# srvk/eesen

Measured on AMD Instinct MI355X. Metric: CTC training frames/sec (whole node), 4x512 BiLSTM, higher is better.
Workload: dtype f32

## Files before the change

### eesen_amd/csrc/kernels.h

```cpp
#pragma once
#include "common.h"

namespace eesen {

struct GemmBound {
  const float* p = nullptr;
  int per_index = 0;
};
void gemm_f32(hipStream_t st, bool a_kc, bool b_kc, int M, int N, int K, float alpha, const float* A, int lda,
              const float* B, int ldb, float beta, float* C, int ldc, const float* bias, float* ws,
              size_t ws_floats, int extra_lds_bytes = 0,
              bool bf16_operands = false,
              GemmBound bound_a = {}, GemmBound bound_b = {});

constexpr int kDefaultGemmMode = 2;
int gemm_mode();
void set_gemm_mode(int mode);
void amax_abs(hipStream_t st, const float* P, long rows, int cols, int ld, float* out);
void amax_abs_accumulate(hipStream_t st, const float* P, long rows, int cols, int ld, float* out);
constexpr int kAmaxBlocks = 512;
void amax_rows_cols(hipStream_t st, const float* P, long rows, int cols, int ld, float* out_rows, float* out_cols, float* ws);

#ifndef EESEN_SHARDS
#define EESEN_SHARDS 8
// ... 29 lines not shown
  int poll_delay = 0;
  int poll_raw = 0;
  unsigned* milestone = nullptr;
  int milestone_step = 0;
  int xcd_map = 1, fwd_mux = 1, bwd_q4 = 1, bwd_ksplit = 1, bwd_mux = 1;
  int fwd_t16_small = 1;
  int fwd_narrow2 = 1;
  int bwd_q4_st8 = 1;
  int fwd_bf16 = 0;
  int fwd_split = 0;
  int fwd_f16 = 0;
  const float* wm_amax = nullptr;
  int bwd_f16 = 0;
  unsigned char* DGH = nullptr;
  float* EX = nullptr;
};
size_t lstm_bwd_planes_ex_floats(const LstmLayerDev& L);
float handoff_flight_ns();
void set_gpu_share(int n);
int gpu_share_value();
void wait_for_word(hipStream_t st, const unsigned* word, unsigned target, unsigned* err, double limit_s = 2.0);
void lstm_fwd_step(hipStream_t st, const LstmLayerDev& L, int step);
void lstm_bwd_step(hipStream_t st, const LstmLayerDev& L, int step, const float* dY, int lddy, float* DG, float* DCF);
bool lstm_fwd_persistent(hipStream_t st, const LstmLayerDev& L, unsigned* cnt, unsigned* err, int spin_limit,
                         unsigned long long* trace = nullptr, hipEvent_t after_reset = nullptr);
void dropout_mask(hipStream_t st, float* out, long rows, int cols, int ld, float p, unsigned long long seed, bool per_column);
void activation_rows(hipStream_t st, bool tanh_, const float* x, int ldx, float* y, int ldy, long rows, int cols);
void activation_diff_rows(hipStream_t st, bool tanh_, const float* y, int ldy, float* d, int ldd, long rows, int cols);
void mul_elements(hipStream_t st, const float* a, int lda, const float* m, int ldm, float* out, int ldo, long rows, int cols);
void lstm_fwd_persistent_geometry(const LstmLayerDev& L, int* nblk, int* nz, int* units_per_wg = nullptr);
// ... 8 lines not shown
  int seq_tile = 0;
  int units = 0;
  int windows = 0;
  int grid[3] = {0, 0, 0};
  int wgs = 0;
  int wgs_per_cu = 0;
  int vgprs = 0, lds = 0;
  int free_vgprs = -1;
  bool light = false;
  int cpw = 0, stq = 0, chunk = 0, xchg = 0;
  const void* fn = nullptr;
};
RecPlan lstm_fwd_plan(const LstmLayerDev& L);
RecPlan lstm_bwd_plan(const LstmLayerDev& L, bool assume_px);
bool lstm_bwd_persistent(hipStream_t st, const LstmLayerDev& L, const float* dY, int lddy, float* DG, unsigned* cnt,
                         unsigned* err, int spin_limit, unsigned long long* trace = nullptr);
void lstm_bias_peep_grads(hipStream_t st, const LstmLayerDev& L, const float* DG, float* bias_grad, float* peep_grad,
                          float* ws, size_t ws_floats);
size_t lstm_bias_peep_ws_floats(int T, int S, int H, int ndir);

void col_sums(hipStream_t st, const float* M, int rows, int cols, int ld, float* out, float* ws, size_t ws_floats);
size_t col_sums_ws_floats(int rows, int cols);

void softmax_rows(hipStream_t st, const float* x, int ldx, float* y, int ldy, int rows, int K);
void log_rows(hipStream_t st, const float* in, int ldi, float* out, int ldo, int rows, int K);
void ctc_alpha_beta(hipStream_t st, const float* logp, int ld, int T, int S, int Lpad, const int* labx, const int* lens,
                    const int* lablens, float* alpha, float* beta, float* pzx, int waves = 0);
int ctc_sweep_waves(int Lpad, int waves = 0);
void ctc_error_diff(hipStream_t st, const float* probs, int ld, int T, int S, int K, int Lpad, int Lmax, const int* lens,
                    const int* lablens, const int* labx, const float* alpha, const float* beta,
                    const float* pzx, float* diff, int ldd);
void log_sub_prior(hipStream_t st, float* m, int ld, int rows, int K, bool apply_log, const float* log_prior, float prior_scale);
void row_argmax(hipStream_t st, const float* m, int ld, int rows, int K, int* ids);
// ... 22 lines not shown
```

### eesen_amd/csrc/lstm.hip

```cpp
#include "kernels.h"

namespace eesen {
namespace {

typedef float f32x4 __attribute__((ext_vector_type(4)));
constexpr int NW = 8;

#ifndef EESEN_RCP
#define EESEN_RCP(x) __builtin_amdgcn_rcpf(x)
#endif
__device__ __forceinline__ float sigmoidf_(float x) { return EESEN_RCP(1.f + __expf(-x)); }
__device__ __forceinline__ float tanhf_(float x) { return 1.f - 2.f * EESEN_RCP(1.f + __expf(2.f * x)); }

__device__ __forceinline__ void ld8(const float* __restrict__ row, int k, int kmax, bool ok, float (&v)[8]) {
  float4 a = make_float4(0.f, 0.f, 0.f, 0.f), b = a;
  if (ok && k < kmax) a = *reinterpret_cast<const float4*>(row + k);
  if (ok && k + 4 < kmax) b = *reinterpret_cast<const float4*>(row + k + 4);
  v[0] = a.x; v[1] = a.y; v[2] = a.z; v[3] = a.w;
  v[4] = b.x; v[5] = b.y; v[6] = b.z; v[7] = b.w;
}

template <int CPW>
__global__ __launch_bounds__(NW * 64) void lstm_fwd_step_kernel(LstmLayerDev L, int step) {
  __shared__ __attribute__((aligned(16))) float red[NW][32][20];
// ... 168 lines not shown
    dcm = dc * L.rmask[cofs];
    if (L.drop_mode == 2) dcx = dcm;
  }
  float df = f * (1.f - f) * (dcx * c_p);
  float di = i * (1.f - i) * (dcm * g);
  float dg = (1.f - g * g) * (dcm * i);
  float carry = dcx * f;
  if (t >= len) { dg = di = df = dob = 0.f; carry = 0.f; }
  *reinterpret_cast<float4*>(DG + gofs) = make_float4(dg, di, df, dob);
  DCF[(size_t)s_e * ldY + dir * H + u_e] = carry;
  asm volatile("" ::"v"(pf.x), "v"(pf.y), "v"(pf.z), "v"(pf.w), "v"(pf1), "v"(pf2));
}

constexpr int RED_RB = 64;

__global__ __launch_bounds__(256) void lstm_bias_peep_pass1(const float* __restrict__ DG, const float* __restrict__ C,
                                                            int R, int S, int H, int ndir, float* __restrict__ ws) {
  __shared__ float sm[4][64][7];
  const int ul = threadIdx.x & 63, rl = threadIdx.x >> 6;
  const int NU = ndir * H;
  const int gu = blockIdx.x * 64 + ul;
  const int rows_per = (R + RED_RB - 1) / RED_RB;
  const int rbeg = blockIdx.y * rows_per, rend = min(R, rbeg + rows_per);
  float acc[7] = {0.f, 0.f, 0.f, 0.f, 0.f, 0.f, 0.f};
  if (gu < NU) {
    const int dir = gu / H;
    const size_t cs_shift = dir == 0 ? 0 : 2 * (size_t)S;
    for (int r = rbeg + rl; r < rend; r += 4) {
      const float4 d = *reinterpret_cast<const float4*>(DG + (size_t)r * NU * 4 + (size_t)gu * 4);
      const float cs = C[((size_t)r + cs_shift) * NU + gu];
      const float c1 = C[((size_t)r + S) * NU + gu];
      acc[0] += d.x; acc[1] += d.y; acc[2] += d.z; acc[3] += d.w;
      acc[4] += d.y * cs; acc[5] += d.z * cs; acc[6] += d.w * c1;
    }
  }
#pragma unroll
  for (int q = 0; q < 7; ++q) sm[rl][ul][q] = acc[q];
  __syncthreads();
  if (rl == 0 && gu < NU) {
#pragma unroll
    for (int q = 0; q < 7; ++q)
      ws[((size_t)blockIdx.y * NU + gu) * 7 + q] = sm[0][ul][q] + sm[1][ul][q] + sm[2][ul][q] + sm[3][ul][q];
  }
}

__global__ __launch_bounds__(256) void lstm_bias_peep_pass2(const float* __restrict__ ws, int H, int ndir,
                                                            float* __restrict__ bias_grad, float* __restrict__ peep_grad) {
  const int NU = ndir * H;
  const int idx = blockIdx.x * blockDim.x + threadIdx.x;
  if (idx >= NU * 7) return;
  const int gu = idx / 7, q = idx % 7;
  float s = 0.f;
  for (int rb = 0; rb < RED_RB; ++rb) s += ws[((size_t)rb * NU + gu) * 7 + q];
  if (q < 4) {
    bias_grad[(size_t)gu * 4 + q] = s;
  } else {
    const int dir = gu / H, u = gu % H;
    peep_grad[((size_t)dir * 3 + (q - 4)) * H + u] = s;
  }
}

__global__ __launch_bounds__(256) void col_sums_pass1(const float* __restrict__ M, int rows, int cols, int ld,
                                                      float* __restrict__ ws) {
  __shared__ float sm[4][64];
  const int cl = threadIdx.x & 63, rl = threadIdx.x >> 6;
  const int c = blockIdx.x * 64 + cl;
  const int rows_per = (rows + RED_RB - 1) / RED_RB;
  const int rbeg = blockIdx.y * rows_per, rend = min(rows, rbeg + rows_per);
  float acc = 0.f;
  if (c < cols)
    for (int r = rbeg + rl; r < rend; r += 4) acc += M[(size_t)r * ld + c];
  sm[rl][cl] = acc;
  __syncthreads();
// ... 18 lines not shown
void lstm_fwd_step(hipStream_t st, const LstmLayerDev& L, int step) {
  dim3 grid(L.H / 4, L.ndir, cdiv(L.S, 32)), block(NW * 64);
  switch (std::min(4, pick_cpw((L.H + 31) / 32))) {
    case 1: hipLaunchKernelGGL(lstm_fwd_step_kernel<1>, grid, block, 0, st, L, step); break;
    case 2: hipLaunchKernelGGL(lstm_fwd_step_kernel<2>, grid, block, 0, st, L, step); break;
    default: hipLaunchKernelGGL(lstm_fwd_step_kernel<4>, grid, block, 0, st, L, step); break;
  }
}

void lstm_bwd_step(hipStream_t st, const LstmLayerDev& L, int step, const float* dY, int lddy, float* DG, float* DCF) {
  dim3 grid(cdiv(L.H, 16), L.ndir, cdiv(L.S, 16)), block(NW * 64);
  if (pick_cpw((4 * L.H + 31) / 32) <= 1) hipLaunchKernelGGL(lstm_bwd_step_kernel<1>, grid, block, 0, st, L, step, dY, lddy, DG, DCF);
  else hipLaunchKernelGGL(lstm_bwd_step_kernel<2>, grid, block, 0, st, L, step, dY, lddy, DG, DCF);
}

size_t lstm_bias_peep_ws_floats(int T, int S, int H, int ndir) { return (size_t)RED_RB * ndir * H * 7; }

void lstm_bias_peep_grads(hipStream_t st, const LstmLayerDev& L, const float* DG, float* bias_grad, float* peep_grad,
                          float* ws, size_t ws_floats) {
  const int NU = L.ndir * L.H, R = L.T * L.S;
  EESEN_REQUIRE(ws_floats >= lstm_bias_peep_ws_floats(L.T, L.S, L.H, L.ndir), EESEN_ERR_INVALID, "reduction workspace too small");
  hipLaunchKernelGGL(lstm_bias_peep_pass1, dim3(cdiv(NU, 64), RED_RB), dim3(256), 0, st, DG, (const float*)L.C, R, L.S,
                     L.H, L.ndir, ws);
  check_launch("lstm_bias_peep_pass1");
  hipLaunchKernelGGL(lstm_bias_peep_pass2, dim3(cdiv(NU * 7, 256)), dim3(256), 0, st, (const float*)ws, L.H, L.ndir,
                     bias_grad, peep_grad);
  check_launch("lstm_bias_peep_pass2");
}

size_t col_sums_ws_floats(int rows, int cols) { return (size_t)RED_RB * cols; }

void col_sums(hipStream_t st, const float* M, int rows, int cols, int ld, float* out, float* ws, size_t ws_floats) {
  EESEN_REQUIRE(ws_floats >= col_sums_ws_floats(rows, cols), EESEN_ERR_INVALID, "reduction workspace too small");
  hipLaunchKernelGGL(col_sums_pass1, dim3(cdiv(cols, 64), RED_RB), dim3(256), 0, st, M, rows, cols, ld, ws);
  check_launch("col_sums_pass1");
  hipLaunchKernelGGL(col_sums_pass2, dim3(cdiv(cols, 256)), dim3(256), 0, st, (const float*)ws, cols, out);
  check_launch("col_sums_pass2");
}

}
```

### eesen_amd/csrc/lstm_persistent.hip

```cpp
#include "kernels.h"

#include <atomic>
#include <map>
#include <mutex>

namespace eesen {
namespace {

typedef float f32x4 __attribute__((ext_vector_type(4)));
constexpr int NW = 8;
constexpr int kSc1 = 16;

#define EESEN_RCP(x) __builtin_amdgcn_rcpf(x)
__device__ __forceinline__ float sigmoidf_(float x) { return EESEN_RCP(1.f + __expf(-x)); }
__device__ __forceinline__ float tanhf_(float x) { return 1.f - 2.f * EESEN_RCP(1.f + __expf(2.f * x)); }

__device__ __forceinline__ __amdgpu_buffer_rsrc_t make_rsrc(const float* base) {
  return __builtin_amdgcn_make_buffer_rsrc(const_cast<float*>(base), 0, 0x7fffffff, 0x00020000);
}
__device__ __forceinline__ float ld1(__amdgpu_buffer_rsrc_t r, unsigned byte_off) {
  return __builtin_bit_cast(float, __builtin_amdgcn_raw_buffer_load_b32(r, byte_off, 0, 0));
}
constexpr int EESEN_POLL_WAVE = 7;
constexpr int EESEN_POLL_SLEEP = 1;
// ... 896 lines not shown
  float dcf = 0.f, dn_i = 0.f, dn_f = 0.f;
  const size_t gcol = (size_t)dir * K4 + u_e * 4;
  const size_t ycol = (size_t)dir * H + u_e;
  float4 gt = make_float4(0.f, 0.f, 0.f, 0.f);
  float dy = 0.f, c_t = 0.f, c_p = 0.f;
  {
    const int t0 = dir == 0 ? T - 1 : 0, tp0 = dir == 0 ? t0 - 1 : t0 + 1;
    if (e_ok) {
      gt = *reinterpret_cast<const float4*>(L.G + (size_t)(t0 * S + s_e) * ldG + gcol);
      dy = dY[(size_t)(t0 * S + s_e) * lddy + ycol];
      c_t = L.C[(size_t)((t0 + 1) * S + s_e) * ldY + ycol];
      c_p = L.C[(size_t)((tp0 + 1) * S + s_e) * ldY + ycol];
    }
  }
  const __amdgpu_buffer_rsrc_t rDG = make_rsrc(DG);
  __syncthreads();
  for (int step = 0; step < T; ++step) {
    const int t = dir == 0 ? T - 1 - step : step;
    const int tn = dir == 0 ? t + 1 : t - 1;
    f32x4 ac[HS][2];
#pragma unroll
    for (int hs = 0; hs < HS; ++hs) { ac[hs][0] = f32x4{0.f, 0.f, 0.f, 0.f}; ac[hs][1] = f32x4{0.f, 0.f, 0.f, 0.f}; }
    f32x4 a4[HS][P];
    const float4 gtc = gt;
    const float dyc = dy, ctc = c_t, cpc = c_p;
    EESEN_STAMP(0);
    if (step > 0) {
      if (wave == EESEN_POLL_WAVE) {
        const bool go = wait_counters(my_cnt, nblk, (unsigned)step, err, spin_limit, lane, L.poll_delay);
        if (lane == 0) s_go = go ? 1 : 0;
// ... 36 lines not shown
              if (h == 0)      { ac[hs][0] = __builtin_amdgcn_mfma_f32_4x4x1f32(a4[hs][p][r], w0[r], ac[hs][0], 3, 0, 0); ac[hs][1] = __builtin_amdgcn_mfma_f32_4x4x1f32(a4[hs][p][r], w1[r], ac[hs][1], 3, 1, 0); }
              else if (h == 1) { ac[hs][0] = __builtin_amdgcn_mfma_f32_4x4x1f32(a4[hs][p][r], w0[r], ac[hs][0], 3, 2, 0); ac[hs][1] = __builtin_amdgcn_mfma_f32_4x4x1f32(a4[hs][p][r], w1[r], ac[hs][1], 3, 3, 0); }
              else if (h == 2) { ac[hs][0] = __builtin_amdgcn_mfma_f32_4x4x1f32(a4[hs][p][r], w0[r], ac[hs][0], 3, 4, 0); ac[hs][1] = __builtin_amdgcn_mfma_f32_4x4x1f32(a4[hs][p][r], w1[r], ac[hs][1], 3, 5, 0); }
              else             { ac[hs][0] = __builtin_amdgcn_mfma_f32_4x4x1f32(a4[hs][p][r], w0[r], ac[hs][0], 3, 6, 0); ac[hs][1] = __builtin_amdgcn_mfma_f32_4x4x1f32(a4[hs][p][r], w1[r], ac[hs][1], 3, 7, 0); }
            }
          }
        }
      }
    }
#pragma unroll
    for (int hs = 0; hs < HS; ++hs)
#pragma unroll
      for (int i = 0; i < 4; ++i) red[wave][hs * 8 + ks * 4 + i][ab * 4 + x] = ac[hs][0][i] + ac[hs][1][i];
    EESEN_STAMP(2);
    __syncthreads();
    if (e_ok) {
      float ra[NW], rb[NW];
#pragma unroll
      for (int w = 0; w < NW; ++w) { ra[w] = red[w][(es >> 2) * 8 + (es & 3)][eu]; rb[w] = red[w][(es >> 2) * 8 + 4 + (es & 3)][eu]; }
      __builtin_amdgcn_sched_barrier(0);
      float dm = dyc;
#pragma unroll
      for (int w = 0; w < NW; ++w) dm += ra[w] + rb[w];
      const float g = gtc.x, i = gtc.y, f = gtc.z, o = gtc.w;
      const float h = tanhf_(ctc);
      const float dh = (1.f - h * h) * (dm * o);
      float dob = o * (1.f - o) * (dm * h);
      const float dc = dh + dcf + dn_i * p_i + dn_f * p_f + dob * p_o;
      float df = f * (1.f - f) * (dc * cpc);
      float di = i * (1.f - i) * (dc * g);
      float dg = (1.f - g * g) * (dc * i);
      float carry = dc * f;
      if (t >= len) { dg = di = df = dob = 0.f; carry = 0.f; }
      const f32x4 out = {dg, di, df, dob};
      __builtin_amdgcn_raw_buffer_store_b128(out, rDG, (unsigned)(((size_t)(t * S + s_e) * ldG + gcol) * 4), 0, kSc1);
      dcf = carry; dn_i = di; dn_f = df;
    }
    EESEN_STAMP(3);
    if (step + 1 < T) {
      if (tid < ST * UW) asm volatile("s_waitcnt vmcnt(0)" ::: "memory");
      __syncthreads();
      EESEN_STAMP(4);
      if (tid == 0) __hip_atomic_fetch_add(my_cnt + (bx & (kShards - 1)) * kShardStride, 1u, __ATOMIC_RELAXED, __HIP_MEMORY_SCOPE_AGENT);
      if (e_ok) {
        const int t2 = dir == 0 ? t - 1 : t + 1, tp2 = dir == 0 ? t2 - 1 : t2 + 1;
        gt = *reinterpret_cast<const float4*>(L.G + (size_t)(t2 * S + s_e) * ldG + gcol);
        dy = dY[(size_t)(t2 * S + s_e) * lddy + ycol];
        c_t = c_p;
        c_p = L.C[(size_t)((tp2 + 1) * S + s_e) * ldY + ycol];
      }
    }
  }
}

__device__ __forceinline__ void px_put(unsigned long long* p, float v, unsigned tag) {
  __hip_atomic_store(p, ((unsigned long long)tag << 32) | (unsigned long long)__float_as_uint(v), __ATOMIC_RELAXED, __HIP_MEMORY_SCOPE_AGENT);
}
template <int KU>
__device__ __forceinline__ void px_load(const unsigned long long* px, int ku, int off, unsigned long long (&w)[KU]) {
#pragma unroll
  for (int src = 0; src < KU; ++src)
    w[src] = src == ku ? 0ull : __hip_atomic_load(px + (size_t)(ku * KU + src) * 256 + off, __ATOMIC_RELAXED, __HIP_MEMORY_SCOPE_AGENT);
}
template <int KU>
__device__ __forceinline__ bool px_take(const unsigned long long* px, int ku, int off, unsigned tag, unsigned* err, int spin_limit,
                                        unsigned long long (&w)[KU], float& sum) {
// ... 1017 lines not shown
  const int ncu = share_of_cus();
  const long blocks16 = (long)cdiv(L.H, 16) * L.ndir * cdiv(L.S, 16);
  if (2 * blocks16 <= ncu && L.S > 8) return 0;
  return (size_t)2 * L.ndir * cdiv(L.S, 16) * (size_t)(L.H / 64) * 4096 * 2;
}

static bool bwd_planes_shape(const LstmLayerDev& L) {
  if (!L.bwd_f16 || !L.bwd_ksplit || L.wm_amax == nullptr) return false;
  const int cpw = (4 * L.H / 4) / (32 * NW);
  return lstm_bwd_ksplit_px_floats(L) != 0 && (cpw == 2 || cpw == 4) && (4 * L.H / 4) % (32 * NW) == 0;
}
size_t lstm_bwd_planes_ex_floats(const LstmLayerDev& L) {
  return bwd_planes_shape(L) ? (size_t)L.T * L.ndir * cdiv(L.S, 16) * (size_t)(L.H / 16) * 16 : 0;
}

RecPlan lstm_bwd_plan(const LstmLayerDev& L0, bool assume_px) {
  RecPlan P;
  const int nch = (4 * L0.H + 31) / 32;
  const int need = (nch + NW - 1) / NW;
  const int ncu = share_of_cus();
  const long blocks16 = (long)cdiv(L0.H, 16) * L0.ndir * cdiv(L0.S, 16);
  const int stile = 2 * blocks16 <= ncu && L0.S > 8 ? 8 : 16;
  P.light = stile == 8;
  if (need > 16 || L0.T < 2) return P;
  if (((size_t)L0.S * L0.ndir * 4 * L0.H * sizeof(float)) % 128 != 0) return P;
  const size_t blk_bytes = (size_t)L0.S * L0.ndir * 4 * L0.H * sizeof(float);
  const long max_blocks = (long)((((size_t)1 << 31) - 1) / blk_bytes);
  if (max_blocks < 3) return P;
  int chunk = (int)std::min<long>(L0.T, max_blocks - 1);
  if (chunk < L0.T) { int p2 = 1; while (p2 * 2 <= chunk) p2 *= 2; chunk = p2; }
// ... 66 lines not shown
    dim3 grid(cdiv(L0.H, 16), L0.ndir, cdiv(Sw, stile));
    if ((size_t)grid.y * grid.z * kShards * kShardStride > (size_t)kCtlHalf) return false;
    return fits(fn, grid, NW * 64);
  };
  const int nwin = pick_windows(L0.S, stile, gfits);
  if (nwin == 0) return P;
  if (nwin > 1 && ((size_t)(L0.S / nwin) * L0.ndir * 4 * L0.H * sizeof(float)) % 128 != 0) return P;
  const dim3 grid(cdiv(L0.H, 16), L0.ndir, cdiv(L0.S / nwin, stile));
  P.kind = kRecBwdGeneric; P.fn = fn; P.cpw = bwd_generic_cpw(need); P.seq_tile = stile; P.units = 16; P.windows = nwin;
  snprintf(P.kernel, sizeof(P.kernel), "lstm_bwd_persistent_kernel<%d,%d,%s>", P.cpw, stile, L0.drop_mode ? "true" : "false");
  plan_resources(P, grid);
  return P;
}

bool lstm_bwd_persistent(hipStream_t st, const LstmLayerDev& L0, const float* dY, int lddy, float* DG, unsigned* cnt,
                         unsigned* err, int spin_limit, unsigned long long* trace) {
  const RecPlan P = lstm_bwd_plan(L0, false);
  if (P.kind == kRecNone) return false;
  const dim3 grid(P.grid[0], P.grid[1], P.grid[2]);
  const Role role{P.grid[0], P.grid[1], P.grid[2], L0.xcd_map};
  int chunk = P.chunk;
  if (P.kind == kRecBwdQ4) {
    LstmLayerDev L = L0;
    L.s_begin = 0; L.s_count = 0;
    EESEN_HIP_CHECK(hipMemsetAsync(cnt, 0, sizeof(unsigned) * grid.y * grid.z * kShards * kShardStride, st));
    plan_launch(st, P, grid, L, dY, lddy, DG, cnt, err, spin_limit, trace, role);
    return true;
  }
  if (P.kind == kRecBwdKsplitMux || P.kind == kRecBwdKsplit) {
    const size_t px_need = lstm_bwd_ksplit_px_floats(L0);
    unsigned long long* px = reinterpret_cast<unsigned long long*>(L0.PX);
    for (int w = 0; w < P.windows; ++w) {
      LstmLayerDev L = L0;
      if (P.kind == kRecBwdKsplitMux) { L.s_begin = 0; L.s_count = 0; }
      else { L.s_count = L0.S / P.windows; L.s_begin = w * L.s_count; }
      const size_t c1 = (size_t)L0.ndir * (P.kind == kRecBwdKsplitMux ? cdiv(L0.S, 16) : (int)grid.z) * 4 * kShards * kShardStride;
      EESEN_HIP_CHECK(hipMemsetAsync(cnt, 0, sizeof(unsigned) * c1, st));
      EESEN_HIP_CHECK(hipMemsetAsync(L.PX, 0, sizeof(float) * px_need, st));
      if (P.kind == kRecBwdKsplitMux) plan_launch(st, P, grid, L, dY, lddy, DG, px, cnt, err, spin_limit, role, chunk);
// ... 16 lines not shown
```

### eesen_amd/csrc/net.cpp

```cpp
#include "net.h"

#include <algorithm>
#include <cmath>
#include <cstdio>
#include <cstring>

namespace eesen {


PhaseTimer::~PhaseTimer() {
  for (auto& s : spans_) {
    (void)hipEventDestroy(s.a);
    (void)hipEventDestroy(s.b);
  }
}
int PhaseTimer::begin(hipStream_t st, int phase) {
  if (!on_) return -1;
  if (used_ == spans_.size()) {
    Span s;
    EESEN_HIP_CHECK(hipEventCreate(&s.a));
    EESEN_HIP_CHECK(hipEventCreate(&s.b));
    spans_.push_back(s);
  }
  spans_[used_].phase = phase;
// ... 72 lines not shown

Net::Net(int dev, void* stream) : device(dev) {
  int n = 0;
  hipError_t e = hipGetDeviceCount(&n);
  if (e != hipSuccess || n <= 0)
    throw Error(EESEN_ERR_HIP, "no HIP device available: this library has no CPU fallback (hipGetDeviceCount: " +
                                   std::string(e == hipSuccess ? "0 devices" : hipGetErrorString(e)) + ")");
  EESEN_REQUIRE(dev >= 0 && dev < n, EESEN_ERR_INVALID, "device index out of range");
  EESEN_HIP_CHECK(hipSetDevice(dev));
  st = reinterpret_cast<hipStream_t>(stream);
  int lo = 0, hi = 0;
  EESEN_HIP_CHECK(hipDeviceGetStreamPriorityRange(&lo, &hi));
  EESEN_HIP_CHECK(hipStreamCreateWithPriority(&st2, hipStreamNonBlocking, lo));
  EESEN_HIP_CHECK(hipEventCreateWithFlags(&ev_rec, hipEventDisableTiming));
  for (auto& e : ev_grad) EESEN_HIP_CHECK(hipEventCreateWithFlags(&e, hipEventDisableTiming));
  EESEN_HIP_CHECK(hipEventCreateWithFlags(&ev_gate_reset, hipEventDisableTiming));
  EESEN_HIP_CHECK(hipEventCreateWithFlags(&ev_gate_done, hipEventDisableTiming));
  tn = Tuning::from_env();
  persistent = tn.persistent;
  gate_fwd = tn.gate_fwd >= 0 ? tn.gate_fwd != 0 : gemm_mode() == 0;
  overlap = tn.overlap >= 0 ? tn.overlap != 0 : persistent != 0;
  spin_limit = tn.spin_limit;
  if (tn.trace) {
    trace.reserve(1280);
    EESEN_HIP_CHECK(hipMemset(trace.p, 0, 1280 * sizeof(unsigned long long)));
  }
  ctl.reserve(kCtlWords);
  EESEN_HIP_CHECK(hipMemset(ctl.p, 0, kCtlWords * sizeof(unsigned)));
  {
    constexpr float kFwdNs = 400.f, kBwdNs = 280.f, kBwdSideNs = 420.f, kRefFlightNs = 400.f;
// ... 37 lines not shown
          ++n;
        }
        if (n) fprintf(stderr, "EESEN_TRACE %s: wait %.0f | A-load+MFMA+reduce %.0f | epilogue %.0f | drain+barrier %.0f | publish->next %.0f ticks/step (%d steps)\n",
                       pass ? "bwd" : "fwd", seg[0] / n, seg[1] / n, seg[2] / n, seg[3] / n, seg[4] / n, n);
      }
  }
  if (lens_pin) (void)hipHostFree(lens_pin);
  if (err_pin) (void)hipHostFree(err_pin);
  if (live_pin) (void)hipHostFree(live_pin);
  for (auto& h : in_stage) { if (h.p) (void)hipHostFree(h.p); if (h.ev) (void)hipEventDestroy(h.ev); }
  if (lens_ev) (void)hipEventDestroy(lens_ev);
  if (err_ev) (void)hipEventDestroy(err_ev);
  if (st2) { (void)hipStreamSynchronize(st2); (void)hipStreamDestroy(st2); }
  if (ev_rec) (void)hipEventDestroy(ev_rec);
  for (auto& e : ev_grad) if (e) (void)hipEventDestroy(e);
  if (ev_gate_reset) (void)hipEventDestroy(ev_gate_reset);
  if (ev_gate_done) (void)hipEventDestroy(ev_gate_done);
  for (auto& e : ev_ready) if (e) (void)hipEventDestroy(e);
  for (auto& e : ev_bucket) if (e) (void)hipEventDestroy(e);
  if (ev_bwd_done) (void)hipEventDestroy(ev_bwd_done);
  if (own_stream) (void)hipStreamDestroy(st);
}

void Net::sync() {
  EESEN_HIP_CHECK(hipSetDevice(device));
  EESEN_HIP_CHECK(hipStreamSynchronize(st));
  wait_buckets_host();
  comm_check_alive(comm);
  check_device_error(true);
}
// ... 632 lines not shown
    need_ws = std::max(need_ws, col_sums_ws_floats(rows, L.dout));
  }
  need_ws = std::max(need_ws, (size_t)16 << 20);
  ws.reserve(need_ws);
  ws_floats = need_ws;
  dA.reserve((size_t)rows * maxdim);
  dB.reserve((size_t)rows * maxdim);
  if (max_g) {
    DGb[0].reserve((size_t)rows * max_g);
    DGb[1].reserve((size_t)rows * max_g);
  }
  if (max_y) DCF.reserve((size_t)S * max_y);
  ws2.reserve(need_ws);
  int dg_slot = 0;
  bool side_pending[2] = {false, false};
  deferred_buckets.clear();
  const bool overlap = overlap_for_minibatch();
  exchange_deferred = comm && exchange_deferred_for_minibatch();
  bucket_log.clear();
  info_bwd_persistent = 0;
  live_valid = comm != nullptr;
  if (comm) {
    comm_check_alive(comm);
    EESEN_HIP_CHECK(hipMemsetD32Async(reinterpret_cast<hipDeviceptr_t>(fresh.p + P), 0x3f800000, 1, st));
  }

  const int Kout = layers.back().dout;
  float* d = dA.p;
  int ld_d = pad4(Kout);
  float* dn = dB.p;
// ... 20 lines not shown
      const Layer& Pv = layers[li - 1];
      if (Pv.is_lstm()) { ldx = Pv.ndir * Pv.H; x = Pv.output(S); }
      else { ldx = pad4(Pv.dout); x = Pv.out.p; }
    }
    const bool want_in = li > 0 || in_diff != nullptr;
    const int ld_n = pad4(L.din);
    float* fr = fresh.p + L.p_off;
    if (L.kind == EESEN_LAYER_SOFTMAX) {
      continue;
    } else if (L.is_activation()) {
      { const int ti_ = timer.begin(st, 4);
      activation_diff_rows(st, L.kind == EESEN_LAYER_TANH, L.out.p, pad4(L.dout), d, ld_d, rows, L.dout);
      timer.end(st, ti_); }
      continue;
    } else if (L.kind == EESEN_LAYER_AFFINE) {
      { const int ti_ = timer.begin(st, 4);
      if (half) measure(d, rows, L.dout, ld_d, L.bd.rows, L.bd.cols);
      if (want_in) {
        if (ld_n != L.din) EESEN_HIP_CHECK(hipMemsetAsync(dn, 0, (size_t)rows * ld_n * sizeof(float), st));
        gemm_f32(st, true, false, rows, L.din, L.dout, 1.f, d, ld_d, params.p + L.p_off + L.off_w, pad4(L.din), 0.f, dn, ld_n,
                 nullptr, nullptr, 0, 0, false, half ? GemmBound{L.bd.rows.p, 1} : GemmBound{}, half ? GemmBound{L.bw.cols.p, 1} : GemmBound{});
      }
      gemm_f32(st, false, false, L.dout, L.din, rows, 1.f, d, ld_d, x, ldx, 0.f, fr + L.off_w, pad4(L.din), nullptr, ws.p, ws_floats, 0, false,
               half ? GemmBound{L.bd.cols.p, 1} : GemmBound{}, x_cols(li));
      col_sums(st, d, rows, L.dout, ld_d, fr + L.off_b, ws.p, ws_floats);
      timer.end(st, ti_); }
      bucket_allreduce(li, st);
    } else {
      const int H = L.H, nd = L.ndir, ldG = nd * 4 * H, ldY = nd * H;
      LstmLayerDev v = lstm_view(*this, L);
      v.poll_delay = overlap ? delay_bwd_side : delay_bwd;
      v.poll_raw = poll_raw;
      if (persistent) {
        const size_t need = lstm_bwd_ksplit_px_floats(v);
        if (need) { bwd_px.reserve(need); v.PX = bwd_px.p; v.px_floats = bwd_px.cap; }
        if (const size_t ex = lstm_bwd_planes_ex_floats(v)) {
          bwd_dgh.reserve((size_t)rows * ldG);
          bwd_ex.reserve(ex);
          v.DGH = reinterpret_cast<unsigned char*>(bwd_dgh.p);
          v.EX = bwd_ex.p;
        }
      }
      EESEN_REQUIRE(in_train || !L.has_dropout(), EESEN_ERR_STATE, "Can't backpropagate a dropout layer in test mode (bilstm-parallel-layer.h:425)");
      if (L.cur_fwd_drop) mul_elements(st, d, ld_d, L.fmask.p, ldY, d, ld_d, rows, ldY);
      float* DGl = DGb[dg_slot].p;
      if (side_pending[dg_slot]) {
        EESEN_HIP_CHECK(hipStreamWaitEvent(st, ev_grad[dg_slot], 0));
        side_pending[dg_slot] = false;
      }
      { const int ti_ = timer.begin(st, 3);
      if (persistent && lstm_bwd_persistent(st, v, d, ld_d, DGl, ctl.p + kCtlHalf, ctl.p + kCtlWords - 1, spin_limit, trace.p ? trace.p + 640 : nullptr))
        ++info_bwd_persistent;
      else
        for (int step = 0; step < T; ++step) lstm_bwd_step(st, v, step, d, ld_d, DGl, DCF.p);
      check_launch("lstm_bwd");
      timer.end(st, ti_); }
      if (half) { const int ti_ = timer.begin(st, 4); measure(DGl, rows, ldG, ldG, L.bd.rows, L.bd.cols); timer.end(st, ti_); }
      EESEN_HIP_CHECK(hipEventRecord(ev_rec, st));
      if (want_in) {
        const int ti_ = timer.begin(st, 4);
        if (ld_n != L.din) EESEN_HIP_CHECK(hipMemsetAsync(dn, 0, (size_t)rows * ld_n * sizeof(float), st));
        gemm_f32(st, true, false, rows, L.din, ldG, 1.f, DGl, ldG, params.p + L.p_off + L.off_wx, pad4(L.din), 0.f, dn, ld_n,
                 nullptr, nullptr, 0, 0, false, half ? GemmBound{L.bd.rows.p, 1} : GemmBound{}, half ? GemmBound{L.bw.cols.p, 1} : GemmBound{});
        timer.end(st, ti_);
        EESEN_HIP_CHECK(hipEventRecord(ev_rec, st));
      }
      hipStream_t sg = overlap ? st2 : st;
      const int side_lds_env = (tn.side_lds_kb >= 0 ? tn.side_lds_kb : (gemm_mode() >= 1 ? 48 : 32)) * 1024;
      bool lstm_below = false;
      for (int lj = 0; lj < li; ++lj) lstm_below |= layers[lj].is_lstm();
      const int side_lds = overlap && lstm_below ? side_lds_env : 0;
      if (overlap) EESEN_HIP_CHECK(hipStreamWaitEvent(st2, ev_rec, 0));
      { const int ti_ = timer.begin(sg, 4);
      gemm_f32(sg, false, false, ldG, L.din, rows, 1.f, DGl, ldG, x, ldx, 0.f, fr + L.off_wx, pad4(L.din), nullptr, ws2.p, need_ws, side_lds, false,
               half ? GemmBound{L.bd.cols.p, 1} : GemmBound{}, x_cols(li));
      for (int dir = 0; dir < nd; ++dir)
        gemm_f32(sg, false, false, 4 * H, H, rows, 1.f, DGl + (size_t)dir * 4 * H, ldG,
                 L.Y.p + (size_t)(dir == 0 ? 0 : 2 * S) * ldY + (size_t)dir * H, ldY, 0.f,
                 fr + L.off_wm + (size_t)dir * 4 * H * H, H, nullptr, ws2.p, need_ws, side_lds, false,
                 half ? GemmBound{L.bd.cols.p + (size_t)dir * 4 * H, 1} : GemmBound{}, half ? bound_one() : GemmBound{});
      lstm_bias_peep_grads(sg, v, DGl, fr + L.off_bias, fr + L.off_peep, ws2.p, need_ws);
      timer.end(sg, ti_); }
      bucket_allreduce(li, sg);
      if (overlap) {
        EESEN_HIP_CHECK(hipEventRecord(ev_grad[dg_slot], st2));
        side_pending[dg_slot] = true;
      }
      dg_slot ^= 1;
    }
    if (want_in) {
      std::swap(d, dn);
      ld_d = ld_n;
    }
  }
  if (in_diff) copy2d(st, d, ld_d, in_diff, ldi, rows, layers[0].din);
  flush_deferred_buckets();
  for (int k = 0; k < 2; ++k)
    if (side_pending[k]) EESEN_HIP_CHECK(hipStreamWaitEvent(st, ev_grad[k], 0));
}

bool Net::overlap_for_minibatch() const {
  bool ov = overlap;
  if (ov && tn.overlap < 0 && persistent)
    for (const Layer& L : layers)
      if (L.is_lstm() && L.H > 320 && L.H <= 512 && S > 32 && !lstm_bwd_plan(lstm_view(*this, L), true).light) ov = false;
  return ov;
}
bool Net::exchange_deferred_for_minibatch() const {
  if (tn.comm_defer >= 0) return tn.comm_defer != 0;
  if (!persistent) return false;
  for (const Layer& L : layers)
    if (L.is_lstm()) {
      const RecPlan bp = lstm_bwd_plan(lstm_view(*this, L), true);
// ... 76 lines not shown
```

### eesen_amd/csrc/net.h

```cpp
#pragma once
#include <string>
#include <vector>

#include "kernels.h"
#include "tuning.h"

namespace eesen {

inline int pad4(int x) { return (x + 3) & ~3; }
constexpr size_t kCtlWords = 2 * kCtlHalf + 32;

struct Layer {
  int kind = 0, din = 0, dout = 0;
  float coef = 1.f, max_grad = 0.f;
  size_t p_off = 0, p_n = 0;
  int H = 0, ndir = 0;
  int din_f = 0, dout_f = 0, Hf = 0;
  int in_nb = 0, in_hf = 0, in_hi = 0, out_nb = 0, out_hf = 0, out_hi = 0;
  int in_col(int d) const { return in_nb ? (d / in_hf) * in_hi + d % in_hf : d; }
  size_t off_wx = 0, off_bias = 0, off_wm = 0, off_peep = 0;
  DevBuf<float> WmT;
  DevBuf<float> G, C, Y;
  DevBuf<float> X;
  size_t off_w = 0, off_b = 0;
// ... 58 lines not shown
  void set_accu(const float* host, long n);
  std::vector<int> lens;
  DevBuf<int> lens_d;
  int T = 0, S = 0, rows = 0;
  bool propagated = false;
  DevBuf<float> input;
  struct HostStage { float* p = nullptr; size_t cap = 0; hipEvent_t ev = nullptr; bool busy = false; } in_stage[2];
  unsigned in_stage_idx = 0;
  const float* out_ptr = nullptr;
  int out_cols = 0, out_ld = 0;
  DevBuf<float> out_f;
  DevBuf<float> DGb[2], DCF, dA, dB, ws, ws2;
  DevBuf<float> bwd_px;
  DevBuf<float> bwd_dgh, bwd_ex;
  hipStream_t st2 = nullptr;
  hipEvent_t ev_rec = nullptr, ev_grad[2] = {nullptr, nullptr};
  bool overlap = true;
  hipEvent_t ev_gate_reset = nullptr, ev_gate_done = nullptr;
  DevBuf<unsigned> mile;
  bool gate_fwd = true;
  bool fwd_bf16 = false;
  bool fwd_bf16_rec = false;
  int info_fwd_bf16 = 0;
  DevBuf<unsigned> ctl;
  Tuning tn;
  int persistent = 1;
  int info_fwd_persistent = 0, info_bwd_persistent = 0, info_lstm_layers = 0;
  int spin_limit = 400000;
  float flight_ns = 0.f;
  int delay_fwd = 61, delay_bwd = 43, delay_bwd_side = 64, poll_raw = 0;
  int recoveries = 0;
// ... 147 lines not shown
```

### eesen_amd/csrc/tuning.h

```cpp
#pragma once
#include <cstdlib>

namespace eesen {

struct Tuning {
  int persistent = 1;
  int overlap = -1, gate_fwd = -1, side_lds_kb = -1;
  int spin_limit = 400000;
  bool spin_limit_set = false;
  int bwd_q4 = 1, bwd_q4_st8 = 1, fwd_narrow2 = 1, fwd_t16_small = 1, bwd_ksplit = 1, fwd_mux = 1, bwd_mux = 1, xcd_map = 1, fwd_mid = 1, fwd_split = 1, fwd_f16 = 1, bwd_f16 = 1;
  int comm_defer = -1;
  int trace = 0;
  bool print_flight = false;
  const char* poll_ns = nullptr;

  static Tuning from_env() {
    Tuning t;
    auto num = [](const char* name, int dflt) {
      const char* e = getenv(name);
      return e && *e ? atoi(e) : dflt;
    };
    t.persistent = num("EESEN_PERSISTENT", 1);
    t.overlap = num("EESEN_OVERLAP", -1);
    t.gate_fwd = num("EESEN_GATE_FWD", -1);
    t.fwd_mid = num("EESEN_FWD_MID", 1);
    t.side_lds_kb = num("EESEN_SIDE_LDS_KB", -1);
    t.spin_limit_set = getenv("EESEN_SPIN_LIMIT") != nullptr;
    t.spin_limit = num("EESEN_SPIN_LIMIT", 400000);
    t.bwd_q4 = num("EESEN_BWD_Q4", 1);
    t.bwd_q4_st8 = num("EESEN_BWD_Q4_ST8", 1);
    t.fwd_narrow2 = num("EESEN_FWD_NARROW2", 1);
    t.fwd_t16_small = num("EESEN_FWD_T16_SMALL", 1);
    t.bwd_ksplit = num("EESEN_BWD_KSPLIT", 1);
    t.fwd_mux = num("EESEN_FWD_MUX", 1);
    t.bwd_mux = num("EESEN_BWD_MUX", 1);
    t.fwd_split = num("EESEN_FWD_SPLIT", 1);
    t.fwd_f16 = num("EESEN_FWD_F16", 1);
    t.bwd_f16 = num("EESEN_BWD_F16", 1);
    t.xcd_map = num("EESEN_XCD_MAP", 1);
    t.comm_defer = num("EESEN_COMM_DEFER", -1);
    t.trace = num("EESEN_TRACE", 0);
    t.print_flight = getenv("EESEN_PRINT_FLIGHT") != nullptr;
    t.poll_ns = getenv("EESEN_POLL_NS");
    return t;
  }
};

}
```

Before: 1.004 million.

## Fuse DG row/col abs-max bounds into backward LSTM kernel and bias reduction

The persistent Q4 backward kernel now computes per-row abs-max partials of the gate gradients using DPP reductions and writes them to a row-bound buffer. A small fold kernel combines these partials into the row bounds, and the bias/peephole reduction produces the column bounds alongside its sums. This replaces the separate measure pass over DG. The affine layer's weight-gradient GEMM, column sums and allreduce are also moved to the side stream when it sits above the LSTMs, with an event that guards later writes to the buffer it reads. The cost is extra work and stores inside the recurrent kernel, plus more cross-stream synchronisation.

```diff
diff --git a/eesen_amd/csrc/kernels.h b/eesen_amd/csrc/kernels.h
--- a/eesen_amd/csrc/kernels.h
+++ b/eesen_amd/csrc/kernels.h
@@ -67,6 +67,7 @@
   int bwd_f16 = 0;
   unsigned char* DGH = nullptr;
   float* EX = nullptr;
+  unsigned* RB = nullptr;
 };
 size_t lstm_bwd_planes_ex_floats(const LstmLayerDev& L);
 float handoff_flight_ns();
@@ -105,9 +106,12 @@
 RecPlan lstm_fwd_plan(const LstmLayerDev& L);
 RecPlan lstm_bwd_plan(const LstmLayerDev& L, bool assume_px);
 bool lstm_bwd_persistent(hipStream_t st, const LstmLayerDev& L, const float* dY, int lddy, float* DG, unsigned* cnt,
-                         unsigned* err, int spin_limit, unsigned long long* trace = nullptr);
+                         unsigned* err, int spin_limit, unsigned long long* trace = nullptr, bool* rb_emitted = nullptr);
+size_t lstm_bwd_row_bound_words(const LstmLayerDev& L);
+inline size_t lstm_bwd_row_bound_ld(long rows) { return ((size_t)rows + 3) & ~(size_t)3; }
+void lstm_bwd_row_bounds_fold(hipStream_t st, const LstmLayerDev& L, float* out_rows);
 void lstm_bias_peep_grads(hipStream_t st, const LstmLayerDev& L, const float* DG, float* bias_grad, float* peep_grad,
-                          float* ws, size_t ws_floats);
+                          float* ws, size_t ws_floats, float* out_cols = nullptr);
 size_t lstm_bias_peep_ws_floats(int T, int S, int H, int ndir);
 
 void col_sums(hipStream_t st, const float* M, int rows, int cols, int ld, float* out, float* ws, size_t ws_floats);
diff --git a/eesen_amd/csrc/lstm.hip b/eesen_amd/csrc/lstm.hip
--- a/eesen_amd/csrc/lstm.hip
+++ b/eesen_amd/csrc/lstm.hip
@@ -206,15 +206,18 @@
 
 constexpr int RED_RB = 64;
 
+template <bool BOUNDS>
 __global__ __launch_bounds__(256) void lstm_bias_peep_pass1(const float* __restrict__ DG, const float* __restrict__ C,
                                                             int R, int S, int H, int ndir, float* __restrict__ ws) {
   __shared__ float sm[4][64][7];
+  __shared__ uint4 smx[BOUNDS ? 4 : 1][BOUNDS ? 64 : 1];
   const int ul = threadIdx.x & 63, rl = threadIdx.x >> 6;
   const int NU = ndir * H;
   const int gu = blockIdx.x * 64 + ul;
   const int rows_per = (R + RED_RB - 1) / RED_RB;
   const int rbeg = blockIdx.y * rows_per, rend = min(R, rbeg + rows_per);
   float acc[7] = {0.f, 0.f, 0.f, 0.f, 0.f, 0.f, 0.f};
+  uint4 cm = make_uint4(0u, 0u, 0u, 0u);
   if (gu < NU) {
     const int dir = gu / H;
     const size_t cs_shift = dir == 0 ? 0 : 2 * (size_t)S;
@@ -224,23 +227,44 @@
       const float c1 = C[((size_t)r + S) * NU + gu];
       acc[0] += d.x; acc[1] += d.y; acc[2] += d.z; acc[3] += d.w;
       acc[4] += d.y * cs; acc[5] += d.z * cs; acc[6] += d.w * c1;
+      if (BOUNDS) {
+        cm.x = max(cm.x, __float_as_uint(d.x) & 0x7fffffffu); cm.y = max(cm.y, __float_as_uint(d.y) & 0x7fffffffu);
+        cm.z = max(cm.z, __float_as_uint(d.z) & 0x7fffffffu); cm.w = max(cm.w, __float_as_uint(d.w) & 0x7fffffffu);
+      }
     }
   }
 #pragma unroll
   for (int q = 0; q < 7; ++q) sm[rl][ul][q] = acc[q];
+  if (BOUNDS) smx[BOUNDS ? rl : 0][BOUNDS ? ul : 0] = cm;
   __syncthreads();
   if (rl == 0 && gu < NU) {
 #pragma unroll
     for (int q = 0; q < 7; ++q)
       ws[((size_t)blockIdx.y * NU + gu) * 7 + q] = sm[0][ul][q] + sm[1][ul][q] + sm[2][ul][q] + sm[3][ul][q];
+    if (BOUNDS) {
+      uint4 m = cm;
+#pragma unroll
+      for (int k = 1; k < 4; ++k) { const uint4 o = smx[BOUNDS ? k : 0][BOUNDS ? ul : 0]; m.x = max(m.x, o.x); m.y = max(m.y, o.y); m.z = max(m.z, o.z); m.w = max(m.w, o.w); }
+      unsigned* wb = reinterpret_cast<unsigned*>(ws) + (size_t)RED_RB * NU * 7;
+      *reinterpret_cast<uint4*>(wb + ((size_t)blockIdx.y * NU + gu) * 4) = m;
+    }
   }
 }
 
 __global__ __launch_bounds__(256) void lstm_bias_peep_pass2(const float* __restrict__ ws, int H, int ndir,
-                                                            float* __restrict__ bias_grad, float* __restrict__ peep_grad) {
+                                                            float* __restrict__ bias_grad, float* __restrict__ peep_grad,
+                                                            unsigned* __restrict__ cols) {
   const int NU = ndir * H;
   const int idx = blockIdx.x * blockDim.x + threadIdx.x;
-  if (idx >= NU * 7) return;
+  if (idx >= NU * 7) {
+    const int c = idx - NU * 7;
+    if (cols == nullptr || c >= NU * 4) return;
+    const unsigned* wb = reinterpret_cast<const unsigned*>(ws) + (size_t)RED_RB * NU * 7;
+    unsigned m = 0u;
+    for (int rb = 0; rb < RED_RB; ++rb) m = max(m, wb[(size_t)rb * NU * 4 + c]);
+    cols[c] = m;
+    return;
+  }
   const int gu = idx / 7, q = idx % 7;
   float s = 0.f;
   for (int rb = 0; rb < RED_RB; ++rb) s += ws[((size_t)rb * NU + gu) * 7 + q];
@@ -249,6 +273,26 @@
   } else {
     const int dir = gu / H, u = gu % H;
     peep_grad[((size_t)dir * 3 + (q - 4)) * H + u] = s;
+  }
+}
+
+__global__ __launch_bounds__(256) void lstm_row_bounds_fold_kernel(const unsigned* __restrict__ part, int np, size_t ld, long rows,
+                                                                   unsigned* __restrict__ out) {
+  const long r = ((long)blockIdx.x * blockDim.x + threadIdx.x) * 4;
+  if (r >= rows) return;
+  uint4 m = make_uint4(0u, 0u, 0u, 0u);
+  for (int p0 = 0; p0 < np; p0 += 8) {
+    uint4 v[8];
+#pragma unroll
+    for (int k = 0; k < 8; ++k) v[k] = p0 + k < np ? *reinterpret_cast<const uint4*>(part + (size_t)(p0 + k) * ld + r) : make_uint4(0u, 0u, 0u, 0u);
+#pragma unroll
+    for (int k = 0; k < 8; ++k) { m.x = max(m.x, v[k].x); m.y = max(m.y, v[k].y); m.z = max(m.z, v[k].z); m.w = max(m.w, v[k].w); }
+  }
+  if (r + 3 < rows) *reinterpret_cast<uint4*>(out + r) = m;
+  else {
+    out[r] = m.x;
+    if (r + 1 < rows) out[r + 1] = m.y;
+    if (r + 2 < rows) out[r + 2] = m.z;
   }
 }
 
@@ -297,18 +341,30 @@
   else hipLaunchKernelGGL(lstm_bwd_step_kernel<2>, grid, block, 0, st, L, step, dY, lddy, DG, DCF);
 }
 
-size_t lstm_bias_peep_ws_floats(int T, int S, int H, int ndir) { return (size_t)RED_RB * ndir * H * 7; }
+size_t lstm_bias_peep_ws_floats(int T, int S, int H, int ndir) { return (size_t)RED_RB * ndir * H * (7 + 4); }
 
 void lstm_bias_peep_grads(hipStream_t st, const LstmLayerDev& L, const float* DG, float* bias_grad, float* peep_grad,
-                          float* ws, size_t ws_floats) {
+                          float* ws, size_t ws_floats, float* out_cols) {
   const int NU = L.ndir * L.H, R = L.T * L.S;
   EESEN_REQUIRE(ws_floats >= lstm_bias_peep_ws_floats(L.T, L.S, L.H, L.ndir), EESEN_ERR_INVALID, "reduction workspace too small");
-  hipLaunchKernelGGL(lstm_bias_peep_pass1, dim3(cdiv(NU, 64), RED_RB), dim3(256), 0, st, DG, (const float*)L.C, R, L.S,
-                     L.H, L.ndir, ws);
+  if (out_cols)
+    hipLaunchKernelGGL(lstm_bias_peep_pass1<true>, dim3(cdiv(NU, 64), RED_RB), dim3(256), 0, st, DG, (const float*)L.C, R, L.S,
+                       L.H, L.ndir, ws);
+  else
+    hipLaunchKernelGGL(lstm_bias_peep_pass1<false>, dim3(cdiv(NU, 64), RED_RB), dim3(256), 0, st, DG, (const float*)L.C, R, L.S,
+                       L.H, L.ndir, ws);
   check_launch("lstm_bias_peep_pass1");
-  hipLaunchKernelGGL(lstm_bias_peep_pass2, dim3(cdiv(NU * 7, 256)), dim3(256), 0, st, (const float*)ws, L.H, L.ndir,
-                     bias_grad, peep_grad);
+  hipLaunchKernelGGL(lstm_bias_peep_pass2, dim3(cdiv(NU * (out_cols ? 11 : 7), 256)), dim3(256), 0, st, (const float*)ws, L.H, L.ndir,
+                     bias_grad, peep_grad, reinterpret_cast<unsigned*>(out_cols));
   check_launch("lstm_bias_peep_pass2");
+}
+
+void lstm_bwd_row_bounds_fold(hipStream_t st, const LstmLayerDev& L, float* out_rows) {
+  const long rows = (long)L.T * L.S;
+  EESEN_REQUIRE(L.RB != nullptr && L.H % 32 == 0, EESEN_ERR_INVALID, "row-bound fold without partials");
+  hipLaunchKernelGGL(lstm_row_bounds_fold_kernel, dim3((unsigned)cdivl(cdivl(rows, 4), 256)), dim3(256), 0, st, (const unsigned*)L.RB,
+                     L.ndir * (L.H / 32), lstm_bwd_row_bound_ld(rows), rows, reinterpret_cast<unsigned*>(out_rows));
+  check_launch("lstm_row_bounds_fold");
 }
 
 size_t col_sums_ws_floats(int rows, int cols) { return (size_t)RED_RB * cols; }
diff --git a/eesen_amd/csrc/lstm_persistent.hip b/eesen_amd/csrc/lstm_persistent.hip
--- a/eesen_amd/csrc/lstm_persistent.hip
+++ b/eesen_amd/csrc/lstm_persistent.hip
@@ -934,6 +934,7 @@
     }
   }
   const __amdgpu_buffer_rsrc_t rDG = make_rsrc(DG);
+  unsigned* const RBp = L.RB ? L.RB + (size_t)(dir * (H / UW) + bx) * ((((size_t)T * S) + 3) & ~(size_t)3) : nullptr;
   __syncthreads();
   for (int step = 0; step < T; ++step) {
     const int t = dir == 0 ? T - 1 - step : step;
@@ -1000,6 +1001,7 @@
       for (int i = 0; i < 4; ++i) red[wave][hs * 8 + ks * 4 + i][ab * 4 + x] = ac[hs][0][i] + ac[hs][1][i];
     EESEN_STAMP(2);
     __syncthreads();
+    unsigned rbm = 0u;
     if (e_ok) {
       float ra[NW], rb[NW];
 #pragma unroll
@@ -1021,9 +1023,18 @@
       const f32x4 out = {dg, di, df, dob};
       __builtin_amdgcn_raw_buffer_store_b128(out, rDG, (unsigned)(((size_t)(t * S + s_e) * ldG + gcol) * 4), 0, kSc1);
       dcf = carry; dn_i = di; dn_f = df;
+      if (RBp) rbm = max(max(__float_as_uint(dg), __float_as_uint(di)), max(__float_as_uint(df), __float_as_uint(dob))) & 0x7fffffffu;
+    }
+    if (RBp && tid < ST * UW) {
+      rbm = max(rbm, (unsigned)__builtin_amdgcn_update_dpp(0, (int)rbm, 0xB1, 0xf, 0xf, false));
+      rbm = max(rbm, (unsigned)__builtin_amdgcn_update_dpp(0, (int)rbm, 0x4E, 0xf, 0xf, false));
+      rbm = max(rbm, (unsigned)__builtin_amdgcn_update_dpp(0, (int)rbm, 0x141, 0xf, 0xf, false));
+      rbm = max(rbm, (unsigned)__builtin_amdgcn_update_dpp(0, (int)rbm, 0x140, 0xf, 0xf, false));
+      rbm = max(rbm, (unsigned)__builtin_amdgcn_update_dpp(0, (int)rbm, 0x142, 0xa, 0xf, false));
     }
     EESEN_STAMP(3);
-    if (step + 1 < T) {
+    const bool more = step + 1 < T;
+    if (more) {
       if (tid < ST * UW) asm volatile("s_waitcnt vmcnt(0)" ::: "memory");
       __syncthreads();
       EESEN_STAMP(4);
@@ -1036,6 +1047,7 @@
         c_p = L.C[(size_t)((tp2 + 1) * S + s_e) * ldY + ycol];
       }
     }
+    if (RBp && e_ok && eu == 16) RBp[t * S + s_e] = rbm;
   }
 }
 
@@ -2083,6 +2095,10 @@
   return bwd_planes_shape(L) ? (size_t)L.T * L.ndir * cdiv(L.S, 16) * (size_t)(L.H / 16) * 16 : 0;
 }
 
+size_t lstm_bwd_row_bound_words(const LstmLayerDev& L) {
+  if (!L.bwd_q4 || L.drop_mode || L.H % 32 != 0 || L.H > 512) return 0;
+  return (size_t)L.ndir * (L.H / 32) * lstm_bwd_row_bound_ld((long)L.T * L.S);
+}
 RecPlan lstm_bwd_plan(const LstmLayerDev& L0, bool assume_px) {
   RecPlan P;
   const int nch = (4 * L0.H + 31) / 32;
@@ -2179,7 +2195,8 @@
 }
 
 bool lstm_bwd_persistent(hipStream_t st, const LstmLayerDev& L0, const float* dY, int lddy, float* DG, unsigned* cnt,
-                         unsigned* err, int spin_limit, unsigned long long* trace) {
+                         unsigned* err, int spin_limit, unsigned long long* trace, bool* rb_emitted) {
+  if (rb_emitted) *rb_emitted = false;
   const RecPlan P = lstm_bwd_plan(L0, false);
   if (P.kind == kRecNone) return false;
   const dim3 grid(P.grid[0], P.grid[1], P.grid[2]);
@@ -2188,6 +2205,7 @@
   if (P.kind == kRecBwdQ4) {
     LstmLayerDev L = L0;
     L.s_begin = 0; L.s_count = 0;
+    if (rb_emitted) *rb_emitted = L.RB != nullptr;
     EESEN_HIP_CHECK(hipMemsetAsync(cnt, 0, sizeof(unsigned) * grid.y * grid.z * kShards * kShardStride, st));
     plan_launch(st, P, grid, L, dY, lddy, DG, cnt, err, spin_limit, trace, role);
     return true;
diff --git a/eesen_amd/csrc/net.cpp b/eesen_amd/csrc/net.cpp
--- a/eesen_amd/csrc/net.cpp
+++ b/eesen_amd/csrc/net.cpp
@@ -110,6 +110,7 @@
   EESEN_HIP_CHECK(hipStreamCreateWithPriority(&st2, hipStreamNonBlocking, lo));
   EESEN_HIP_CHECK(hipEventCreateWithFlags(&ev_rec, hipEventDisableTiming));
   for (auto& e : ev_grad) EESEN_HIP_CHECK(hipEventCreateWithFlags(&e, hipEventDisableTiming));
+  EESEN_HIP_CHECK(hipEventCreateWithFlags(&ev_aff, hipEventDisableTiming));
   EESEN_HIP_CHECK(hipEventCreateWithFlags(&ev_gate_reset, hipEventDisableTiming));
   EESEN_HIP_CHECK(hipEventCreateWithFlags(&ev_gate_done, hipEventDisableTiming));
   tn = Tuning::from_env();
@@ -177,6 +178,7 @@
   if (st2) { (void)hipStreamSynchronize(st2); (void)hipStreamDestroy(st2); }
   if (ev_rec) (void)hipEventDestroy(ev_rec);
   for (auto& e : ev_grad) if (e) (void)hipEventDestroy(e);
+  if (ev_aff) (void)hipEventDestroy(ev_aff);
   if (ev_gate_reset) (void)hipEventDestroy(ev_gate_reset);
   if (ev_gate_done) (void)hipEventDestroy(ev_gate_done);
   for (auto& e : ev_ready) if (e) (void)hipEventDestroy(e);
@@ -839,6 +841,13 @@
   ws2.reserve(need_ws);
   int dg_slot = 0;
   bool side_pending[2] = {false, false};
+  const float* aff_reads = nullptr;
+  auto before_write = [&](const float* buf) {
+    if (aff_reads != buf) return;
+    EESEN_HIP_CHECK(hipStreamWaitEvent(st, ev_aff, 0));
+    aff_reads = nullptr;
+  };
+  bool aff_unjoined = false;
   deferred_buckets.clear();
   const bool overlap = overlap_for_minibatch();
   exchange_deferred = comm && exchange_deferred_for_minibatch();
@@ -889,18 +898,36 @@
       timer.end(st, ti_); }
       continue;
     } else if (L.kind == EESEN_LAYER_AFFINE) {
+      bool lstm_above = false, lstm_below = false;
+      for (size_t lj = li + 1; lj < layers.size(); ++lj) lstm_above |= layers[lj].is_lstm();
+      for (int lj = 0; lj < li; ++lj) lstm_below |= layers[lj].is_lstm();
+      const bool side = overlap && !lstm_above && lstm_below;
+      hipStream_t sa = side ? st2 : st;
+      float* wsa = side ? ws2.p : ws.p;
       { const int ti_ = timer.begin(st, 4);
       if (half) measure(d, rows, L.dout, ld_d, L.bd.rows, L.bd.cols);
       if (want_in) {
+        before_write(dn);
         if (ld_n != L.din) EESEN_HIP_CHECK(hipMemsetAsync(dn, 0, (size_t)rows * ld_n * sizeof(float), st));
         gemm_f32(st, true, false, rows, L.din, L.dout, 1.f, d, ld_d, params.p + L.p_off + L.off_w, pad4(L.din), 0.f, dn, ld_n,
                  nullptr, nullptr, 0, 0, false, half ? GemmBound{L.bd.rows.p, 1} : GemmBound{}, half ? GemmBound{L.bw.cols.p, 1} : GemmBound{});
       }
-      gemm_f32(st, false, false, L.dout, L.din, rows, 1.f, d, ld_d, x, ldx, 0.f, fr + L.off_w, pad4(L.din), nullptr, ws.p, ws_floats, 0, false,
+      timer.end(st, ti_); }
+      if (side) {
+        EESEN_HIP_CHECK(hipEventRecord(ev_rec, st));
+        EESEN_HIP_CHECK(hipStreamWaitEvent(st2, ev_rec, 0));
+      }
+      { const int ti_ = timer.begin(sa, 4);
+      gemm_f32(sa, false, false, L.dout, L.din, rows, 1.f, d, ld_d, x, ldx, 0.f, fr + L.off_w, pad4(L.din), nullptr, wsa, ws_floats, 0, false,
                half ? GemmBound{L.bd.cols.p, 1} : GemmBound{}, x_cols(li));
-      col_sums(st, d, rows, L.dout, ld_d, fr + L.off_b, ws.p, ws_floats);
-      timer.end(st, ti_); }
-      bucket_allreduce(li, st);
+      col_sums(sa, d, rows, L.dout, ld_d, fr + L.off_b, wsa, ws_floats);
+      timer.end(sa, ti_); }
+      bucket_allreduce(li, sa);
+      if (side) {
+        EESEN_HIP_CHECK(hipEventRecord(ev_aff, st2));
+        aff_reads = d;
+        aff_unjoined = true;
+      }
     } else {
       const int H = L.H, nd = L.ndir, ldG = nd * 4 * H, ldY = nd * H;
       LstmLayerDev v = lstm_view(*this, L);
@@ -916,7 +943,12 @@
           v.EX = bwd_ex.p;
         }
       }
+      bool rb_emitted = false;
+      if (persistent && half && tn.bwd_bounds) {
+        if (const size_t words = lstm_bwd_row_bound_words(v)) { bwd_rb.reserve(words); v.RB = bwd_rb.p; }
+      }
       EESEN_REQUIRE(in_train || !L.has_dropout(), EESEN_ERR_STATE, "Can't backpropagate a dropout layer in test mode (bilstm-parallel-layer.h:425)");
+      if (L.cur_fwd_drop) { before_write(d); }
       if (L.cur_fwd_drop) mul_elements(st, d, ld_d, L.fmask.p, ldY, d, ld_d, rows, ldY);
       float* DGl = DGb[dg_slot].p;
       if (side_pending[dg_slot]) {
@@ -924,16 +956,26 @@
         side_pending[dg_slot] = false;
       }
       { const int ti_ = timer.begin(st, 3);
-      if (persistent && lstm_bwd_persistent(st, v, d, ld_d, DGl, ctl.p + kCtlHalf, ctl.p + kCtlWords - 1, spin_limit, trace.p ? trace.p + 640 : nullptr))
+      if (persistent && lstm_bwd_persistent(st, v, d, ld_d, DGl, ctl.p + kCtlHalf, ctl.p + kCtlWords - 1, spin_limit, trace.p ? trace.p + 640 : nullptr, &rb_emitted))
         ++info_bwd_persistent;
       else
         for (int step = 0; step < T; ++step) lstm_bwd_step(st, v, step, d, ld_d, DGl, DCF.p);
       check_launch("lstm_bwd");
       timer.end(st, ti_); }
-      if (half) { const int ti_ = timer.begin(st, 4); measure(DGl, rows, ldG, ldG, L.bd.rows, L.bd.cols); timer.end(st, ti_); }
+      if (half) {
+        const int ti_ = timer.begin(st, 4);
+        if (!rb_emitted) measure(DGl, rows, ldG, ldG, L.bd.rows, L.bd.cols);
+        else {
+          L.bd.rows.reserve((size_t)rows);
+          L.bd.cols.reserve((size_t)ldG);
+          if (want_in) lstm_bwd_row_bounds_fold(st, v, L.bd.rows.p);
+        }
+        timer.end(st, ti_);
+      }
       EESEN_HIP_CHECK(hipEventRecord(ev_rec, st));
       if (want_in) {
         const int ti_ = timer.begin(st, 4);
+        before_write(dn);
         if (ld_n != L.din) EESEN_HIP_CHECK(hipMemsetAsync(dn, 0, (size_t)rows * ld_n * sizeof(float), st));
         gemm_f32(st, true, false, rows, L.din, ldG, 1.f, DGl, ldG, params.p + L.p_off + L.off_wx, pad4(L.din), 0.f, dn, ld_n,
                  nullptr, nullptr, 0, 0, false, half ? GemmBound{L.bd.rows.p, 1} : GemmBound{}, half ? GemmBound{L.bw.cols.p, 1} : GemmBound{});
@@ -947,6 +989,8 @@
       const int side_lds = overlap && lstm_below ? side_lds_env : 0;
       if (overlap) EESEN_HIP_CHECK(hipStreamWaitEvent(st2, ev_rec, 0));
       { const int ti_ = timer.begin(sg, 4);
+      const bool fused_cols = half && rb_emitted;
+      if (fused_cols) lstm_bias_peep_grads(sg, v, DGl, fr + L.off_bias, fr + L.off_peep, ws2.p, need_ws, L.bd.cols.p);
       gemm_f32(sg, false, false, ldG, L.din, rows, 1.f, DGl, ldG, x, ldx, 0.f, fr + L.off_wx, pad4(L.din), nullptr, ws2.p, need_ws, side_lds, false,
                half ? GemmBound{L.bd.cols.p, 1} : GemmBound{}, x_cols(li));
       for (int dir = 0; dir < nd; ++dir)
@@ -954,12 +998,13 @@
                  L.Y.p + (size_t)(dir == 0 ? 0 : 2 * S) * ldY + (size_t)dir * H, ldY, 0.f,
                  fr + L.off_wm + (size_t)dir * 4 * H * H, H, nullptr, ws2.p, need_ws, side_lds, false,
                  half ? GemmBound{L.bd.cols.p + (size_t)dir * 4 * H, 1} : GemmBound{}, half ? bound_one() : GemmBound{});
-      lstm_bias_peep_grads(sg, v, DGl, fr + L.off_bias, fr + L.off_peep, ws2.p, need_ws);
+      if (!fused_cols) lstm_bias_peep_grads(sg, v, DGl, fr + L.off_bias, fr + L.off_peep, ws2.p, need_ws);
       timer.end(sg, ti_); }
       bucket_allreduce(li, sg);
       if (overlap) {
         EESEN_HIP_CHECK(hipEventRecord(ev_grad[dg_slot], st2));
         side_pending[dg_slot] = true;
+        aff_unjoined = false;
       }
       dg_slot ^= 1;
     }
@@ -972,6 +1017,7 @@
   flush_deferred_buckets();
   for (int k = 0; k < 2; ++k)
     if (side_pending[k]) EESEN_HIP_CHECK(hipStreamWaitEvent(st, ev_grad[k], 0));
+  if (aff_unjoined) EESEN_HIP_CHECK(hipStreamWaitEvent(st, ev_aff, 0));
 }
 
 bool Net::overlap_for_minibatch() const {
diff --git a/eesen_amd/csrc/net.h b/eesen_amd/csrc/net.h
--- a/eesen_amd/csrc/net.h
+++ b/eesen_amd/csrc/net.h
@@ -96,7 +96,9 @@
   DevBuf<float> bwd_px;
   DevBuf<float> bwd_dgh, bwd_ex;
   hipStream_t st2 = nullptr;
+  DevBuf<unsigned> bwd_rb;
   hipEvent_t ev_rec = nullptr, ev_grad[2] = {nullptr, nullptr};
+  hipEvent_t ev_aff = nullptr;
   bool overlap = true;
   hipEvent_t ev_gate_reset = nullptr, ev_gate_done = nullptr;
   DevBuf<unsigned> mile;
diff --git a/eesen_amd/csrc/tuning.h b/eesen_amd/csrc/tuning.h
--- a/eesen_amd/csrc/tuning.h
+++ b/eesen_amd/csrc/tuning.h
@@ -8,7 +8,7 @@
   int overlap = -1, gate_fwd = -1, side_lds_kb = -1;
   int spin_limit = 400000;
   bool spin_limit_set = false;
-  int bwd_q4 = 1, bwd_q4_st8 = 1, fwd_narrow2 = 1, fwd_t16_small = 1, bwd_ksplit = 1, fwd_mux = 1, bwd_mux = 1, xcd_map = 1, fwd_mid = 1, fwd_split = 1, fwd_f16 = 1, bwd_f16 = 1;
+  int bwd_q4 = 1, bwd_q4_st8 = 1, fwd_narrow2 = 1, fwd_t16_small = 1, bwd_ksplit = 1, fwd_mux = 1, bwd_mux = 1, xcd_map = 1, bwd_bounds = 1, fwd_mid = 1, fwd_split = 1, fwd_f16 = 1, bwd_f16 = 1;
   int comm_defer = -1;
   int trace = 0;
   bool print_flight = false;
@@ -38,6 +38,7 @@
     t.fwd_f16 = num("EESEN_FWD_F16", 1);
     t.bwd_f16 = num("EESEN_BWD_F16", 1);
     t.xcd_map = num("EESEN_XCD_MAP", 1);
+    t.bwd_bounds = num("EESEN_BWD_BOUNDS", 1);
     t.comm_defer = num("EESEN_COMM_DEFER", -1);
     t.trace = num("EESEN_TRACE", 0);
     t.print_flight = getenv("EESEN_PRINT_FLIGHT") != nullptr;
```

New measurement: 929,600. 0.926x the previous value.
